# qgallouedec/deep_rl

Hardware: NVIDIA B200
Metric: PPO env-steps/sec (rollout+update) CartPole-v1 (higher is better)
Workload: dtype bf16

## Files before the change

deep_rl_b200/csrc/drl_env.cuh:

```cuda
#pragma once
#include "drl_common.cuh"

namespace drl {

template <int KIND> struct EnvSpec;
template <> struct EnvSpec<DRL_ENV_CARTPOLE> { static constexpr int O = 4, A = 2, OP = 4; };
template <> struct EnvSpec<DRL_ENV_ACROBOT>  { static constexpr int O = 6, A = 3, OP = 8; };
template <> struct EnvSpec<DRL_ENV_MOUNTAINCAR> { static constexpr int O = 2, A = 3, OP = 4; };

struct EnvLane {
    double s[4];
    int elapsed;
    float ep_ret;
    int ep_len;
};

__device__ __forceinline__ bool cartpole_physics(double (&s)[4], int action) {
    const double gravity = 9.8, masspole = 0.1, total_mass = 0.1 + 1.0, length = 0.5;
    const double polemass_length = 0.1 * 0.5, force_mag = 10.0, tau = 0.02;
    const double theta_thr = 12.0 * 2.0 * 3.14159265358979323846 / 360.0, x_thr = 2.4;
    double x = s[0], x_dot = s[1], th = s[2], th_dot = s[3];
    double force = action == 1 ? force_mag : -force_mag;
    double sinth, costh;
    sincos(th, &sinth, &costh);
    double temp = (force + polemass_length * (th_dot * th_dot) * sinth) / total_mass;
    double thacc = (gravity * sinth - costh * temp) / (length * (4.0 / 3.0 - masspole * (costh * costh) / total_mass));
    double xacc = temp - polemass_length * thacc * costh / total_mass;
    x = x + tau * x_dot;
    x_dot = x_dot + tau * xacc;
    th = th + tau * th_dot;
    th_dot = th_dot + tau * thacc;
    s[0] = x; s[1] = x_dot; s[2] = th; s[3] = th_dot;
    return (x < -x_thr) || (x > x_thr) || (th < -theta_thr) || (th > theta_thr);
}

__device__ __forceinline__ bool mountaincar_physics(double (&s)[4], int action) {
    double position = s[0], velocity = s[1];
    velocity = velocity + ((double)(action - 1) * 0.001 + cos(3.0 * position) * (-0.0025));
    velocity = fmin(fmax(velocity, -0.07), 0.07);
    position = position + velocity;
    position = fmin(fmax(position, -1.2), 0.6);
    if (position == -1.2 && velocity < 0.0) velocity = 0.0;
    s[0] = position; s[1] = velocity;
    return position >= 0.5 && velocity >= 0.0;
}

__device__ __forceinline__ void acrobot_dsdt(const double (&y)[4], double torque, double (&d)[4]) {
    const double m1 = 1.0, m2 = 1.0, l1 = 1.0, lc1 = 0.5, lc2 = 0.5, I1 = 1.0, I2 = 1.0, g = 9.8;
    const double PI = 3.14159265358979323846;
    double th1 = y[0], th2 = y[1], dth1 = y[2], dth2 = y[3];
    double s2, c2;
    sincos(th2, &s2, &c2);
    double d1 = m1 * (lc1 * lc1) + m2 * (l1 * l1 + lc2 * lc2 + 2.0 * l1 * lc2 * c2) + I1 + I2;
    double d2 = m2 * (lc2 * lc2 + l1 * lc2 * c2) + I2;
    double phi2 = m2 * lc2 * g * cos(th1 + th2 - PI / 2.0);
    double phi1 = -m2 * l1 * lc2 * (dth2 * dth2) * s2 - 2.0 * m2 * l1 * lc2 * dth2 * dth1 * s2 +
                  (m1 * lc1 + m2 * l1) * g * cos(th1 - PI / 2.0) + phi2;
    double ddth2 = (torque + d2 / d1 * phi1 - m2 * l1 * lc2 * (dth1 * dth1) * s2 - phi2) /
                   (m2 * (lc2 * lc2) + I2 - (d2 * d2) / d1);
    double ddth1 = -(d2 * ddth2 + phi1) / d1;
    d[0] = dth1; d[1] = dth2; d[2] = ddth1; d[3] = ddth2;
}

__device__ __forceinline__ double wrap_pi(double x) {
    const double PI = 3.14159265358979323846;
    const double diff = PI - (-PI);
    while (x > PI) x = x - diff;
    while (x < -PI) x = x + diff;
    return x;
}

__device__ __forceinline__ bool acrobot_physics(double (&s)[4], int action, float& reward) {
    const double PI = 3.14159265358979323846;
    const double dt = 0.2, dt2 = dt / 2.0;
    double torque = (double)action - 1.0;
    double k1[4], k2[4], k3[4], k4[4], yt[4];
    acrobot_dsdt(s, torque, k1);
#pragma unroll
    for (int i = 0; i < 4; ++i) yt[i] = s[i] + dt2 * k1[i];
    acrobot_dsdt(yt, torque, k2);
#pragma unroll
    for (int i = 0; i < 4; ++i) yt[i] = s[i] + dt2 * k2[i];
    acrobot_dsdt(yt, torque, k3);
#pragma unroll
    for (int i = 0; i < 4; ++i) yt[i] = s[i] + dt * k3[i];
    acrobot_dsdt(yt, torque, k4);
    double ns[4];
#pragma unroll
    for (int i = 0; i < 4; ++i) ns[i] = s[i] + dt / 6.0 * (k1[i] + 2.0 * k2[i] + 2.0 * k3[i] + k4[i]);
    ns[0] = wrap_pi(ns[0]);
    ns[1] = wrap_pi(ns[1]);
    ns[2] = fmin(fmax(ns[2], -4.0 * PI), 4.0 * PI);
    ns[3] = fmin(fmax(ns[3], -9.0 * PI), 9.0 * PI);
#pragma unroll
    for (int i = 0; i < 4; ++i) s[i] = ns[i];
    bool terminal = (-cos(ns[0]) - cos(ns[1] + ns[0])) > 1.0;
    reward = terminal ? 0.0f : -1.0f;
    return terminal;
}

template <int KIND>
__device__ __forceinline__ void env_observation(const double (&s)[4], float (&obs)[EnvSpec<KIND>::OP]) {
    if constexpr (KIND == DRL_ENV_CARTPOLE) {
#pragma unroll
        for (int i = 0; i < 4; ++i) obs[i] = (float)s[i];
    } else if constexpr (KIND == DRL_ENV_MOUNTAINCAR) {
        obs[0] = (float)s[0]; obs[1] = (float)s[1]; obs[2] = 0.0f; obs[3] = 0.0f;
    } else {
        double s1, c1, s2, c2;
        sincos(s[0], &s1, &c1);
        sincos(s[1], &s2, &c2);
        obs[0] = (float)c1; obs[1] = (float)s1; obs[2] = (float)c2; obs[3] = (float)s2;
        obs[4] = (float)s[2]; obs[5] = (float)s[3]; obs[6] = 0.0f; obs[7] = 0.0f;
    }
}

template <int KIND>
__device__ __forceinline__ void env_reset_state(double (&s)[4], uint64_t seed, uint32_t gid, uint64_t step) {
    uint4 o = philox_seeded(seed, gid, (uint32_t)step, (uint32_t)(step >> 32), TAG_RESET);
    if constexpr (KIND == DRL_ENV_MOUNTAINCAR) {
        s[0] = -0.6 + 0.2 * u01_f64(o.x);
        s[1] = 0.0; s[2] = 0.0; s[3] = 0.0;
        return;
    }
    const double half = KIND == DRL_ENV_CARTPOLE ? 0.05 : 0.1;
    s[0] = -half + (2.0 * half) * u01_f64(o.x);
    s[1] = -half + (2.0 * half) * u01_f64(o.y);
    s[2] = -half + (2.0 * half) * u01_f64(o.z);
    s[3] = -half + (2.0 * half) * u01_f64(o.w);
}

template <int KIND>
__device__ __forceinline__ bool env_physics(double (&s)[4], int action, float& reward) {
    if constexpr (KIND == DRL_ENV_CARTPOLE) { reward = 1.0f; return cartpole_physics(s, action); }
    else if constexpr (KIND == DRL_ENV_MOUNTAINCAR) { reward = -1.0f; return mountaincar_physics(s, action); }
    else { return acrobot_physics(s, action, reward); }
}

template <int KIND>
__device__ __forceinline__ bool env_after_physics(EnvLane& e, bool term, float reward, uint64_t seed, uint32_t gid, uint64_t step,
                                                  int max_episode_steps, const drl_ep_log_t& log);

template <int KIND>
__device__ __forceinline__ bool env_step(EnvLane& e, int action, float& reward, uint64_t seed, uint32_t gid,
                                         uint64_t step, int max_episode_steps, const drl_ep_log_t& log) {
    const bool term = env_physics<KIND>(e.s, action, reward);
    return env_after_physics<KIND>(e, term, reward, seed, gid, step, max_episode_steps, log);
}

template <int KIND>
__device__ __forceinline__ bool env_after_physics(EnvLane& e, bool term, float reward, uint64_t seed, uint32_t gid, uint64_t step,
                                                  int max_episode_steps, const drl_ep_log_t& log) {
    e.elapsed += 1;
    bool done = term || (e.elapsed >= max_episode_steps);
    e.ep_ret = e.ep_ret + reward;
    e.ep_len += 1;
    if (log.count != nullptr) {
        const unsigned active = __activemask();
        const unsigned dmask = __ballot_sync(active, done);
        if (dmask != 0u) {
            const int lane = (int)(threadIdx.x & 31u);
            const int leader = __ffs(dmask) - 1;
            double sr = 0.0, sl = 0.0;
            for (unsigned bits = dmask; bits != 0u; bits &= bits - 1u) {
                const int b = __ffs(bits) - 1;
                sr += (double)__shfl_sync(active, e.ep_ret, b);
                sl += (double)__shfl_sync(active, e.ep_len, b);
            }
            uint32_t base = 0;
            if (lane == leader) {
                base = atomicAdd(log.count, (uint32_t)__popc(dmask));
                if (log.sum_ret) atomicAdd(log.sum_ret, sr);
                if (log.sum_len) atomicAdd(log.sum_len, sl);
            }
            base = __shfl_sync(active, base, leader);
            if (done) {
                const uint32_t slot = base + (uint32_t)__popc(dmask & ((1u << lane) - 1u));
                if (slot < log.cap && log.entries) {
                    drl_ep_entry_t en;
                    en.step = step; en.env = gid; en.ret = e.ep_ret; en.len = e.ep_len; en.pad = 0u;
                    log.entries[slot] = en;
                }
            }
        }
    }
    if (done) {
        env_reset_state<KIND>(e.s, seed, gid, step);
        e.elapsed = 0; e.ep_ret = 0.0f; e.ep_len = 0;
    }
    return done;
}

__device__ __forceinline__ void env_load(EnvLane& e, const drl_env_t& env, int n) {
    const int N = env.num_envs;
#pragma unroll
    for (int i = 0; i < 4; ++i) e.s[i] = env.state[(size_t)i * N + n];
    e.elapsed = env.elapsed[n]; e.ep_ret = env.ep_ret[n]; e.ep_len = env.ep_len[n];
}
__device__ __forceinline__ void env_store(const EnvLane& e, const drl_env_t& env, int n) {
    const int N = env.num_envs;
#pragma unroll
    for (int i = 0; i < 4; ++i) env.state[(size_t)i * N + n] = e.s[i];
    env.elapsed[n] = e.elapsed; env.ep_ret[n] = e.ep_ret; env.ep_len[n] = e.ep_len;
}

}
```

deep_rl_b200/csrc/rollout_tc.cu:

```cuda
#include "drl_env.cuh"
#include "drl_pack.cuh"
#include "drl_tc_common.cuh"

namespace drl {

int check_env(const drl_env_t* env);
drl_ep_log_t log_or_empty(const drl_ep_log_t* log);

#ifdef DRL_ROLLOUT_STAMPS
__device__ long long g_ro_dbg[1024];
#define RO_STAMP(ev) do { if (blockIdx.x == 0 && lane == 0 && t >= 8 && t < 12 && (warp == 0 || warp == 5)) g_ro_dbg[(warp == 0 ? 0 : 512) + (t - 8) * 16 + (ev)] = clock64(); } while (0)
#else
#define RO_STAMP(ev) do { } while (0)
#endif
enum : uint32_t { RB_FWD = 1, RB_ROW0 = 2, RB_ROW1 = 6, RB_L1 = 10 };

template <int O, int A>
struct RoTcSmem {
    using P = Packed<O, A>;
    static constexpr int W_BYTES = (P::TC_END - P::TC_W2) * 4;
    static constexpr int OFF_W = 0;
    static constexpr int OFF_H1 = (OFF_W + W_BYTES + 1023) / 1024 * 1024;
    static constexpr int OFF_OBS = OFF_H1 + 32768;
    static constexpr int OBS_BYTES = TC_TILE * P::OW * 4 > 4096 ? TC_TILE * P::OW * 4 : 4096;
    static constexpr int OFF_XCH = OFF_OBS + OBS_BYTES;
    static constexpr int OFF_ST = OFF_XCH + 32 * TC_TILE * 4;
    static constexpr int OFF_CAND = OFF_ST + TC_TILE * 32;
    static constexpr int OFF_BAR = OFF_CAND + 3 * TC_TILE * 32 + 3 * TC_TILE * 8;
    static constexpr int TOTAL = OFF_BAR + 64 + 1024;
};

constexpr int RO_ENV_WARPS = 4;
constexpr int RO_THREADS = TC_THREADS + 32 * RO_ENV_WARPS;

template <int KIND, int REP>
__global__ void __launch_bounds__(RO_THREADS, 1) rollout_tc_kernel(drl_env_t env, const float* __restrict__ packed, int T,
                                                                   uint64_t step0, drl_rollout_buf_t buf, drl_ep_log_t log, const drl_ctrl_t* __restrict__ ctrl) {
    if (ctrl != nullptr) step0 = ctrl->env_step;
    using SP = EnvSpec<KIND>;
    constexpr int O = SP::O, A = SP::A, OP = SP::OP;
    using P = Packed<O, A>;
    using S = RoTcSmem<O, A>;
    constexpr int OW = P::OW;
    constexpr int ROWS = TC_TILE / REP;
    constexpr int QG = 4 / REP;
    constexpr int UPT = HU / REP;
    constexpr bool SPECULATE = KIND != DRL_ENV_ACROBOT;
    static_assert(OW == OP, "obs stride");
    static_assert(REP == 1 || REP == 2 || REP == 4, "replication factor");
    extern __shared__ unsigned char smem_raw[];
    unsigned char* sm = smem_raw + ((1024u - (smem_u32(smem_raw) & 1023u)) & 1023u);
    unsigned char* tW2 = sm + S::OFF_W;
    const float* sW1 = reinterpret_cast<const float*>(sm + S::OFF_W + 2 * H * H * 2);
    const float* sB1 = sW1 + 2 * H * OW;
    const float* sB2 = sB1 + 2 * H;
    const float* sW4 = sB2 + 2 * H;
    const float* sB4 = sW4 + (A + 1) * H;
    unsigned char* tH1 = sm + S::OFF_H1;
    float* obs_s = reinterpret_cast<float*>(sm + S::OFF_OBS);
    float* xch = reinterpret_cast<float*>(sm + S::OFF_XCH);
    double* st_s = reinterpret_cast<double*>(sm + S::OFF_ST);
    double* cand_s = reinterpret_cast<double*>(sm + S::OFF_CAND);
    float2* cand_rt = reinterpret_cast<float2*>(sm + S::OFF_CAND + 3 * TC_TILE * 32);
    uint64_t* bars = reinterpret_cast<uint64_t*>(sm + S::OFF_BAR);
    uint32_t* slot = reinterpret_cast<uint32_t*>(bars + 3);
    unsigned char* tW1B = reinterpret_cast<unsigned char*>(const_cast<float*>(sB4 + 4));
    unsigned char* tOBS = sm + S::OFF_OBS;

    const int tid = threadIdx.x, warp = tid >> 5, lane = tid & 31;
    const bool is_mma_warp = warp == TC_COMPUTE / 32;

    if (tid == 0) {
        mbar_init(bars, 1);
        mbar_init(bars + 1, 1);
        mbar_init(bars + 2, 1);
        mbar_fence_init();
    }
    if (is_mma_warp) umma::tmem_alloc(slot, 128);
    umma::fence_before_sync();
    __syncthreads();
    umma::fence_after_sync();
    if (tid == 0) {
        mbar_expect_tx(bars, (uint32_t)S::W_BYTES);
        const char* src = reinterpret_cast<const char*>(packed + P::TC_W2);
        for (uint32_t off = 0; off < (uint32_t)S::W_BYTES; off += 16384u) {
            const uint32_t n = (uint32_t)S::W_BYTES - off < 16384u ? (uint32_t)S::W_BYTES - off : 16384u;
            bulk_g2s(sm + S::OFF_W + off, src + off, n, bars);
        }
    }
    const uint32_t tmem = *slot;
    mbar_wait(bars, 0);

    if (is_mma_warp) {
        const uint32_t aW2 = smem_u32(tW2), aH1 = smem_u32(tH1);
        constexpr uint32_t ID_FWD = umma::make_idesc(128, 64, false, false);
        const uint32_t aW1B = smem_u32(tW1B), aOBS = smem_u32(tOBS);
        constexpr uint32_t ID_L1 = umma::make_idesc(128, 64, false, false);
        for (int t = 0; t <= T; ++t) {
            if (REP == 1) {
                named_bar_sync(RB_L1, 128 + 32);
                umma::fence_after_sync();
                if (umma::elect_one()) {
#pragma unroll
                    for (int n2 = 0; n2 < 2; ++n2)
                        umma::mma(tmem + n2 * 64, umma::make_desc(aOBS, 2048, 128, umma::LAYOUT_NONE),
                                  umma::make_desc(aW1B + n2 * 2048, 1024, 128, umma::LAYOUT_NONE), ID_L1, 0u);
                    umma::commit(bars + 2);
                }
                __syncwarp();
            }
            named_bar_sync(RB_FWD, TC_THREADS);
            umma::fence_after_sync();
            if (umma::elect_one()) {
#pragma unroll
                for (int n2 = 0; n2 < 2; ++n2)
#pragma unroll
                    for (int kb = 0; kb < 4; ++kb)
                        umma::mma(tmem + n2 * 64, umma::make_desc(aH1 + n2 * 16384 + kb * 32, 16, 1024, umma::LAYOUT_SW128),
                                  umma::make_desc(aW2 + n2 * 8192 + kb * 32, 16, 1024, umma::LAYOUT_SW128), ID_FWD, kb > 0);
                umma::commit(bars + 1);
            }
            __syncwarp();
        }
        umma::fence_before_sync();
        __syncthreads();
        umma::tmem_dealloc(tmem, 128);
        return;
    }

    if (warp > TC_COMPUTE / 32) {
        const int eg = warp - TC_COMPUTE / 32 - 1;
        if (eg < ROWS / 32) {
            const int er_e = eg * 32 + lane;
            const bool live = blockIdx.x * ROWS + er_e < env.num_envs;
            for (int t = 0; t <= T; ++t) {
                named_bar_sync(RB_ROW0 + eg, 128 * REP + 32);
                if (SPECULATE && t < T && live) {
                    const double2* sp = reinterpret_cast<const double2*>(st_s + er_e * 4);
                    const double2 s01 = sp[0], s23 = sp[1];
#pragma unroll
                    for (int a = 0; a < A; ++a) {
                        double cs[4] = {s01.x, s01.y, s23.x, s23.y};
                        float creward;
                        const bool cterm = env_physics<KIND>(cs, a, creward);
                        double2* cp = reinterpret_cast<double2*>(cand_s + ((size_t)a * TC_TILE + er_e) * 4);
                        cp[0] = make_double2(cs[0], cs[1]);
                        cp[1] = make_double2(cs[2], cs[3]);
                        cand_rt[a * TC_TILE + er_e] = make_float2(creward, cterm ? 1.0f : 0.0f);
                    }
                }
                named_bar_arrive(RB_ROW1 + eg, 128 * REP + 32);
            }
        }
        umma::fence_before_sync();
        __syncthreads();
        return;
    }

    const int q = warp & 3, half = (warp >> 2) & 1, net = (warp >> 3) & 1;
    const int grp = q % QG, replica = q / QG;
    const int er = grp * 32 + lane;
    const int u0 = half * HU + replica * UPT;
    const uint32_t trow = tmem + ((uint32_t)(q * 32) << 16);
    const int wrow0 = net == 0 ? 0 : A;
    const int nheads = net == 0 ? A : 1;
    const bool owner_warp = net == 0 && half == 0 && replica == 0;
    const int N = env.num_envs;
    const int n = blockIdx.x * ROWS + er;
    const bool own = owner_warp && n < N;
    const uint32_t gid = env.env_gid0 + (uint32_t)n;
    constexpr int NSLOT = 2 * REP;

    EnvLane e;
    e.s[0] = e.s[1] = e.s[2] = e.s[3] = 0.0; e.elapsed = 0; e.ep_ret = 0.0f; e.ep_len = 0;
    if (own) env_load(e, env, n);
    float lp_diff = 0.0f, lp_sum = 1.0f;

    for (int t = 0; t <= T; ++t) {
        RO_STAMP(0);

        if (owner_warp) {
            float obs[OP];
#pragma unroll
            for (int i = 0; i < OP; ++i) obs[i] = 0.0f;
            if (own) {
                env_observation<KIND>(e.s, obs);
                float4* o4 = reinterpret_cast<float4*>(buf.obs + ((size_t)t * N + n) * OP);
#pragma unroll
                for (int qq = 0; qq < OP / 4; ++qq) o4[qq] = make_float4(obs[4 * qq], obs[4 * qq + 1], obs[4 * qq + 2], obs[4 * qq + 3]);
                double2* sp = reinterpret_cast<double2*>(st_s + er * 4);
                sp[0] = make_double2(e.s[0], e.s[1]);
                sp[1] = make_double2(e.s[2], e.s[3]);
            }
            if (REP == 1) {
                float o16[16];
#pragma unroll
                for (int i = 0; i < 16; ++i) o16[i] = 0.0f;
#pragma unroll
                for (int i = 0; i < O; ++i) {
                    const float hi = __bfloat162float(__float2bfloat16_rn(obs[i]));
                    o16[i] = hi;
                    o16[8 + i] = obs[i] - hi;
                }
                o16[O] = 1.0f;
                umma::store_row_ns16(tOBS, TC_TILE, er, o16);
                umma::fence_proxy_async();
                umma::fence_before_sync();
                named_bar_arrive(RB_L1, 128 + 32);
            } else {
#pragma unroll
                for (int i = 0; i < OP; ++i) {
                    const float hi = __bfloat162float(__float2bfloat16_rn(obs[i]));
                    obs[i] = hi + __bfloat162float(__float2bfloat16_rn(obs[i] - hi));
                }
#pragma unroll
                for (int qq = 0; qq < OP / 4; ++qq)
                    *reinterpret_cast<float4*>(obs_s + er * OW + 4 * qq) = make_float4(obs[4 * qq], obs[4 * qq + 1], obs[4 * qq + 2], obs[4 * qq + 3]);
            }
        }
        RO_STAMP(1);
        named_bar_sync(RB_ROW0 + grp, 128 * REP + 32);
        RO_STAMP(2);

        if (REP == 1) {
            mbar_wait(bars + 2, (uint32_t)t & 1u);
            umma::fence_after_sync();
            float h[UPT];
            umma::ldn<UPT>(trow + net * 64 + u0, h);
#pragma unroll
            for (int j = 0; j < UPT; ++j) h[j] = tanh_mufu(h[j]);
#pragma unroll
            for (int c = 0; c < UPT / 8; ++c) {
                uint4 ch;
                ch.x = umma::pack_bf16(h[8 * c + 0], h[8 * c + 1]);
                ch.y = umma::pack_bf16(h[8 * c + 2], h[8 * c + 3]);
                ch.z = umma::pack_bf16(h[8 * c + 4], h[8 * c + 5]);
                ch.w = umma::pack_bf16(h[8 * c + 6], h[8 * c + 7]);
                *reinterpret_cast<uint4*>(tH1 + net * 16384 + umma::sw128_off(q * 32 + lane, u0 / 8 + c)) = ch;
            }
        } else {
            float x[OW];
#pragma unroll
            for (int qq = 0; qq < OW / 4; ++qq) {
                const float4 v4 = *reinterpret_cast<const float4*>(obs_s + er * OW + 4 * qq);
                x[4 * qq] = v4.x; x[4 * qq + 1] = v4.y; x[4 * qq + 2] = v4.z; x[4 * qq + 3] = v4.w;
            }
            float h[UPT];
            const float* w1 = sW1 + (net * H + u0) * OW;
            const float* b1 = sB1 + net * H + u0;
#pragma unroll
            for (int k4 = 0; k4 < UPT / 4; ++k4) {
                const float4 bb = *reinterpret_cast<const float4*>(b1 + 4 * k4);
                const float bv[4] = {bb.x, bb.y, bb.z, bb.w};
#pragma unroll
                for (int j = 0; j < 4; ++j) {
                    const int kk = 4 * k4 + j;
                    float z = bv[j];
#pragma unroll
                    for (int qq = 0; qq < OW / 4; ++qq) {
                        const float4 w = *reinterpret_cast<const float4*>(w1 + kk * OW + 4 * qq);
                        z = fmaf(x[4 * qq + 3], w.w, fmaf(x[4 * qq + 2], w.z, fmaf(x[4 * qq + 1], w.y, fmaf(x[4 * qq], w.x, z))));
                    }
                    h[kk] = tanh_mufu(z);
                }
            }
            uint4 ch[UPT / 8];
#pragma unroll
            for (int c = 0; c < UPT / 8; ++c) {
                ch[c].x = umma::pack_bf16(h[8 * c + 0], h[8 * c + 1]);
                ch[c].y = umma::pack_bf16(h[8 * c + 2], h[8 * c + 3]);
                ch[c].z = umma::pack_bf16(h[8 * c + 4], h[8 * c + 5]);
                ch[c].w = umma::pack_bf16(h[8 * c + 6], h[8 * c + 7]);
            }
#pragma unroll
            for (int rp = 0; rp < REP; ++rp) {
                const int row = (rp * QG + grp) * 32 + lane;
#pragma unroll
                for (int c = 0; c < UPT / 8; ++c)
                    *reinterpret_cast<uint4*>(tH1 + net * 16384 + umma::sw128_off(row, u0 / 8 + c)) = ch[c];
            }
        }
        RO_STAMP(3);
        umma::fence_proxy_async();
        umma::fence_before_sync();
        named_bar_arrive(RB_FWD, TC_THREADS);
        RO_STAMP(4);

        uint4 rr = make_uint4(0u, 0u, 0u, 0u);
        if (own) {
            if (t > 0) buf.logp[(size_t)(t - 1) * N + n] = __fsub_rn(lp_diff, logf(lp_sum));
            if (t < T) {
                const uint64_t step = step0 + (uint64_t)t;
                rr = philox_seeded(env.seed, gid, (uint32_t)step, (uint32_t)(step >> 32), TAG_ACTION);
            }
        }

        mbar_wait(bars + 1, (uint32_t)t & 1u);
        umma::fence_after_sync();
        RO_STAMP(5);
        {
            float h[UPT];
            umma::ldn<UPT>(trow + net * 64 + u0, h);
            const float* b2 = sB2 + net * H + u0;
#pragma unroll
            for (int k4 = 0; k4 < UPT / 4; ++k4) {
                const float4 bb = *reinterpret_cast<const float4*>(b2 + 4 * k4);
                h[4 * k4 + 0] = tanh_mufu(h[4 * k4 + 0] + bb.x);
                h[4 * k4 + 1] = tanh_mufu(h[4 * k4 + 1] + bb.y);
                h[4 * k4 + 2] = tanh_mufu(h[4 * k4 + 2] + bb.z);
                h[4 * k4 + 3] = tanh_mufu(h[4 * k4 + 3] + bb.w);
            }
#pragma unroll
            for (int a = 0; a < A; ++a) {
                if (a < nheads) {
                    const float* w = sW4 + (wrow0 + a) * H + u0;
                    float s0 = 0.f, s1 = 0.f, s2 = 0.f, s3 = 0.f;
#pragma unroll
                    for (int k4 = 0; k4 < UPT / 4; ++k4) {
                        const float4 ww = *reinterpret_cast<const float4*>(w + 4 * k4);
                        s0 = fmaf(h[4 * k4 + 0], ww.x, s0);
                        s1 = fmaf(h[4 * k4 + 1], ww.y, s1);
                        s2 = fmaf(h[4 * k4 + 2], ww.z, s2);
                        s3 = fmaf(h[4 * k4 + 3], ww.w, s3);
                    }
                    const int j = half * REP + replica;
                    const int sl = net == 0 ? j * A + a : NSLOT * A + j;
                    xch[sl * TC_TILE + er] = (s0 + s1) + (s2 + s3);
                }
            }
        }
        RO_STAMP(6);
        umma::fence_before_sync();
        named_bar_sync(RB_ROW1 + grp, 128 * REP + 32);
        RO_STAMP(7);

        if (own) {
            const size_t i0 = (size_t)t * N + n;
            float v = xch[(NSLOT * A) * TC_TILE + er];
#pragma unroll
            for (int j = 1; j < NSLOT; ++j) v += xch[(NSLOT * A + j) * TC_TILE + er];
            buf.val[i0] = v + sB4[A];
            if (t < T) {
                float l[A];
#pragma unroll
                for (int a = 0; a < A; ++a) {
                    float sacc = xch[a * TC_TILE + er];
#pragma unroll
                    for (int j = 1; j < NSLOT; ++j) sacc += xch[(j * A + a) * TC_TILE + er];
                    l[a] = sacc + sB4[a];
                }
                if (buf.logits != nullptr) {
#pragma unroll
                    for (int a = 0; a < A; ++a) buf.logits[i0 * A + a] = l[a];
                }
                RO_STAMP(8);
                const uint64_t step = step0 + (uint64_t)t;
                RO_STAMP(9);
                const int act = sample_categorical_split<A>(l, u01_f32(rr.x), lp_diff, lp_sum);
                RO_STAMP(10);
                buf.act[i0] = (uint8_t)act;
                float reward;
                bool term;
                if (SPECULATE) {
                    const double2* cp = reinterpret_cast<const double2*>(cand_s + ((size_t)act * TC_TILE + er) * 4);
                    const double2 c01 = cp[0], c23 = cp[1];
                    e.s[0] = c01.x; e.s[1] = c01.y; e.s[2] = c23.x; e.s[3] = c23.y;
                    const float2 rt = cand_rt[act * TC_TILE + er];
                    reward = rt.x; term = rt.y != 0.0f;
                } else {
                    term = env_physics<KIND>(e.s, act, reward);
                }
                const bool done = env_after_physics<KIND>(e, term, reward, env.seed, gid, step, env.max_episode_steps, log);
                buf.rew[i0 + N] = reward;
                buf.done[i0 + N] = done ? 1 : 0;
                RO_STAMP(11);
            }
        }
    }
    if (own) env_store(e, env, n);
    umma::fence_before_sync();
    __syncthreads();
}

template <int KIND, int REP>
static int launch_rollout_tc_rep(const drl_env_t& env, const float* packed, int T, uint64_t step0, const drl_rollout_buf_t& buf,
                                 const drl_ep_log_t& log, cudaStream_t st, const drl_ctrl_t* ctrl) {
    using SP = EnvSpec<KIND>;
    const int smem = RoTcSmem<SP::O, SP::A>::TOTAL;
    DRL_CUDA(cudaFuncSetAttribute(rollout_tc_kernel<KIND, REP>, cudaFuncAttributeMaxDynamicSharedMemorySize, smem));
    constexpr int ROWS = TC_TILE / REP;
    const int blocks = (env.num_envs + ROWS - 1) / ROWS;
    rollout_tc_kernel<KIND, REP><<<blocks, RO_THREADS, smem, st>>>(env, packed, T, step0, buf, log, ctrl);
    DRL_LAUNCH_CHECK("rollout_tc_kernel");
    return DRL_OK;
}

template <int KIND>
static int launch_rollout_tc_kind(const drl_env_t& env, const float* packed, int T, uint64_t step0, const drl_rollout_buf_t& buf,
                                  const drl_ep_log_t& log, cudaStream_t st, const drl_ctrl_t* ctrl) {
    const int sms = sm_count();
    int rows = 128;
    if ((env.num_envs + 127) / 128 < sms) rows = (env.num_envs + 63) / 64 <= sms ? 64 : 128;
    if ((env.num_envs + 63) / 64 < sms && (env.num_envs + 31) / 32 <= sms) rows = 32;
    const char* ov = getenv("DRL_ROLLOUT_ROWS");
    if (ov) { const int v = atoi(ov); if (v == 32 || v == 64 || v == 128) rows = v; }
    if (rows == 32) return launch_rollout_tc_rep<KIND, 4>(env, packed, T, step0, buf, log, st, ctrl);
    if (rows == 64) return launch_rollout_tc_rep<KIND, 2>(env, packed, T, step0, buf, log, st, ctrl);
    return launch_rollout_tc_rep<KIND, 1>(env, packed, T, step0, buf, log, st, ctrl);
}

int launch_rollout_tc(const drl_env_t& env, const float* packed, int T, uint64_t step0, const drl_rollout_buf_t& buf,
                      const drl_ep_log_t& log, cudaStream_t st, const drl_ctrl_t* ctrl) {
    if (env.kind == DRL_ENV_CARTPOLE) return launch_rollout_tc_kind<DRL_ENV_CARTPOLE>(env, packed, T, step0, buf, log, st, ctrl);
    if (env.kind == DRL_ENV_MOUNTAINCAR) return launch_rollout_tc_kind<DRL_ENV_MOUNTAINCAR>(env, packed, T, step0, buf, log, st, ctrl);
    return launch_rollout_tc_kind<DRL_ENV_ACROBOT>(env, packed, T, step0, buf, log, st, ctrl);
}

}

#ifdef DRL_ROLLOUT_STAMPS
extern "C" int drl_debug_rollout_stamps(long long* host_out) {
    return cudaMemcpyFromSymbol(host_out, drl::g_ro_dbg, sizeof(long long) * 1024) == cudaSuccess ? 0 : 1;
}
#endif
```

Before: 545.1 million.

## Speculatively run forward pass on all candidate next states in REP=4 rollout

For CartPole and MountainCar with 32-row tiles, the env warps now precompute the next state for every possible action. They write each candidate observation to shared memory, and the MMA warp then runs layer 2 for all candidates at once into a larger TMEM allocation. Once the action is sampled, compute warps just select the matching hidden row, which takes env physics and layer 1 off the serial per-step critical path. Env warps are split into three roles: sampling, candidate stepping, and bookkeeping/log writes. The cost is NC times more layer-1/MMA work, more shared memory and TMEM, and extra barriers.

```diff
diff --git a/deep_rl_b200/csrc/drl_env.cuh b/deep_rl_b200/csrc/drl_env.cuh
--- a/deep_rl_b200/csrc/drl_env.cuh
+++ b/deep_rl_b200/csrc/drl_env.cuh
@@ -148,11 +148,7 @@
     return env_after_physics<KIND>(e, term, reward, seed, gid, step, max_episode_steps, log);
 }
 
-template <int KIND>
-__device__ __forceinline__ bool env_after_physics(EnvLane& e, bool term, float reward, uint64_t seed, uint32_t gid, uint64_t step,
-                                                  int max_episode_steps, const drl_ep_log_t& log) {
-    e.elapsed += 1;
-    bool done = term || (e.elapsed >= max_episode_steps);
+__device__ __forceinline__ void env_record_step(EnvLane& e, bool done, float reward, uint32_t gid, uint64_t step, const drl_ep_log_t& log) {
     e.ep_ret = e.ep_ret + reward;
     e.ep_len += 1;
     if (log.count != nullptr) {
@@ -184,10 +180,28 @@
             }
         }
     }
+    if (done) { e.ep_ret = 0.0f; e.ep_len = 0; }
+}
+
+template <int KIND>
+__device__ __forceinline__ bool env_after_physics(EnvLane& e, bool term, float reward, uint64_t seed, uint32_t gid, uint64_t step,
+                                                  int max_episode_steps, const drl_ep_log_t& log) {
+    e.elapsed += 1;
+    const bool done = term || (e.elapsed >= max_episode_steps);
+    env_record_step(e, done, reward, gid, step, log);
     if (done) {
         env_reset_state<KIND>(e.s, seed, gid, step);
-        e.elapsed = 0; e.ep_ret = 0.0f; e.ep_len = 0;
-    }
+        e.elapsed = 0;
+    }
+    return done;
+}
+
+template <int KIND>
+__device__ __forceinline__ bool env_next_state(double (&s)[4], int action, int elapsed, int max_episode_steps, uint64_t seed,
+                                               uint32_t gid, uint64_t step, float& reward) {
+    const bool term = env_physics<KIND>(s, action, reward);
+    const bool done = term || (elapsed + 1 >= max_episode_steps);
+    if (done) env_reset_state<KIND>(s, seed, gid, step);
     return done;
 }
 
diff --git a/deep_rl_b200/csrc/rollout_tc.cu b/deep_rl_b200/csrc/rollout_tc.cu
--- a/deep_rl_b200/csrc/rollout_tc.cu
+++ b/deep_rl_b200/csrc/rollout_tc.cu
@@ -9,25 +9,30 @@
 
 #ifdef DRL_ROLLOUT_STAMPS
 __device__ long long g_ro_dbg[1024];
-#define RO_STAMP(ev) do { if (blockIdx.x == 0 && lane == 0 && t >= 8 && t < 12 && (warp == 0 || warp == 5)) g_ro_dbg[(warp == 0 ? 0 : 512) + (t - 8) * 16 + (ev)] = clock64(); } while (0)
+#define RO_STAMP(ev) do { if (blockIdx.x == 0 && lane == 0 && t >= 8 && t < 12 && (warp == 0 || warp == RO_STAMP_W2 || (SPEC && warp == RO_STAMP_W2 + 1))) g_ro_dbg[(warp == 0 ? 0 : 512) + (t - 8) * 16 + (ev)] = clock64(); } while (0)
 #else
 #define RO_STAMP(ev) do { } while (0)
 #endif
-enum : uint32_t { RB_FWD = 1, RB_ROW0 = 2, RB_ROW1 = 6, RB_L1 = 10 };
-
-template <int O, int A>
+enum : uint32_t { RB_FWD = 1, RB_ROW0 = 2, RB_ROW1 = 6, RB_L1 = 10, RB_ACT = 11 };
+
+template <int KIND, int REP>
+constexpr int ro_cands() { return KIND != DRL_ENV_ACROBOT && REP == 4 ? EnvSpec<KIND>::A : 1; }
+
+template <int O, int A, int NC>
 struct RoTcSmem {
     using P = Packed<O, A>;
     static constexpr int W_BYTES = (P::TC_END - P::TC_W2) * 4;
     static constexpr int OFF_W = 0;
     static constexpr int OFF_H1 = (OFF_W + W_BYTES + 1023) / 1024 * 1024;
-    static constexpr int OFF_OBS = OFF_H1 + 32768;
-    static constexpr int OBS_BYTES = TC_TILE * P::OW * 4 > 4096 ? TC_TILE * P::OW * 4 : 4096;
+    static constexpr int OFF_OBS = OFF_H1 + NC * 32768;
+    static constexpr int OBS_BYTES = NC > 1 ? 2 * NC * TC_TILE * P::OW * 4
+                                   : TC_TILE * P::OW * 4 > 4096 ? TC_TILE * P::OW * 4 : 4096;
     static constexpr int OFF_XCH = OFF_OBS + OBS_BYTES;
     static constexpr int OFF_ST = OFF_XCH + 32 * TC_TILE * 4;
     static constexpr int OFF_CAND = OFF_ST + TC_TILE * 32;
-    static constexpr int OFF_BAR = OFF_CAND + 3 * TC_TILE * 32 + 3 * TC_TILE * 8;
+    static constexpr int OFF_BAR = OFF_CAND + (NC > 1 ? 2 : 1) * (3 * TC_TILE * 32 + 3 * TC_TILE * 8);
     static constexpr int TOTAL = OFF_BAR + 64 + 1024;
+    static_assert(TOTAL <= 227 * 1024, "shared memory of one CTA");
 };
 
 constexpr int RO_ENV_WARPS = 4;
@@ -40,13 +45,18 @@
     using SP = EnvSpec<KIND>;
     constexpr int O = SP::O, A = SP::A, OP = SP::OP;
     using P = Packed<O, A>;
-    using S = RoTcSmem<O, A>;
+    constexpr int NC = ro_cands<KIND, REP>();
+    constexpr bool SPEC = NC > 1;
+    using S = RoTcSmem<O, A, NC>;
     constexpr int OW = P::OW;
     constexpr int ROWS = TC_TILE / REP;
     constexpr int QG = 4 / REP;
     constexpr int UPT = HU / REP;
     constexpr bool SPECULATE = KIND != DRL_ENV_ACROBOT;
     static_assert(OW == OP, "obs stride");
+    constexpr uint32_t TMEM_COLS = NC == 1 ? 128u : NC == 2 ? 256u : 512u;
+    constexpr int RO_STAMP_W2 = SPEC ? TC_COMPUTE / 32 + 1 : 5;
+    (void)RO_STAMP_W2;
     static_assert(REP == 1 || REP == 2 || REP == 4, "replication factor");
     extern __shared__ unsigned char smem_raw[];
     unsigned char* sm = smem_raw + ((1024u - (smem_u32(smem_raw) & 1023u)) & 1023u);
@@ -76,7 +86,7 @@
         mbar_init(bars + 2, 1);
         mbar_fence_init();
     }
-    if (is_mma_warp) umma::tmem_alloc(slot, 128);
+    if (is_mma_warp) umma::tmem_alloc(slot, TMEM_COLS);
     umma::fence_before_sync();
     __syncthreads();
     umma::fence_after_sync();
@@ -113,43 +123,205 @@
             umma::fence_after_sync();
             if (umma::elect_one()) {
 #pragma unroll
-                for (int n2 = 0; n2 < 2; ++n2)
-#pragma unroll
-                    for (int kb = 0; kb < 4; ++kb)
-                        umma::mma(tmem + n2 * 64, umma::make_desc(aH1 + n2 * 16384 + kb * 32, 16, 1024, umma::LAYOUT_SW128),
-                                  umma::make_desc(aW2 + n2 * 8192 + kb * 32, 16, 1024, umma::LAYOUT_SW128), ID_FWD, kb > 0);
+                for (int c = 0; c < NC; ++c)
+#pragma unroll
+                    for (int n2 = 0; n2 < 2; ++n2)
+#pragma unroll
+                        for (int kb = 0; kb < 4; ++kb)
+                            umma::mma(tmem + c * 128 + n2 * 64, umma::make_desc(aH1 + c * 32768 + n2 * 16384 + kb * 32, 16, 1024, umma::LAYOUT_SW128),
+                                      umma::make_desc(aW2 + n2 * 8192 + kb * 32, 16, 1024, umma::LAYOUT_SW128), ID_FWD, kb > 0);
                 umma::commit(bars + 1);
             }
             __syncwarp();
         }
         umma::fence_before_sync();
         __syncthreads();
-        umma::tmem_dealloc(tmem, 128);
+        umma::tmem_dealloc(tmem, TMEM_COLS);
         return;
     }
 
+    constexpr int NSLOT = 2 * REP;
+    constexpr uint32_t N_ACT = 128 * REP + 3 * 32;
+    const int N = env.num_envs;
+
+    auto round_hi_lo = [](float (&obs)[OP]) {
+#pragma unroll
+        for (int i = 0; i < OP; ++i) {
+            const float hi = __bfloat162float(__float2bfloat16_rn(obs[i]));
+            obs[i] = hi + __bfloat162float(__float2bfloat16_rn(obs[i] - hi));
+        }
+    };
+    auto store_obs_row = [](float* dst, const float (&obs)[OP]) {
+#pragma unroll
+        for (int qq = 0; qq < OP / 4; ++qq)
+            reinterpret_cast<float4*>(dst)[qq] = make_float4(obs[4 * qq], obs[4 * qq + 1], obs[4 * qq + 2], obs[4 * qq + 3]);
+    };
+    auto head_value = [&](int r) {
+        float v = xch[(NSLOT * A) * TC_TILE + r];
+#pragma unroll
+        for (int j = 1; j < NSLOT; ++j) v += xch[(NSLOT * A + j) * TC_TILE + r];
+        return v + sB4[A];
+    };
+    auto head_logits = [&](int r, float (&l)[A]) {
+#pragma unroll
+        for (int a = 0; a < A; ++a) {
+            float sacc = xch[a * TC_TILE + r];
+#pragma unroll
+            for (int j = 1; j < NSLOT; ++j) sacc += xch[(j * A + a) * TC_TILE + r];
+            l[a] = sacc + sB4[a];
+        }
+    };
+
     if (warp > TC_COMPUTE / 32) {
         const int eg = warp - TC_COMPUTE / 32 - 1;
-        if (eg < ROWS / 32) {
+        if constexpr (SPEC) {
+            const int n = blockIdx.x * ROWS + lane;
+            const bool live = blockIdx.x * ROWS + lane < env.num_envs;
+            const uint32_t gid = env.env_gid0 + (uint32_t)n;
+            int* sel_s = reinterpret_cast<int*>(st_s);
+            double2* cst = reinterpret_cast<double2*>(cand_s);
+            float2* crt = reinterpret_cast<float2*>(cand_s + 2 * NC * TC_TILE * 4);
+            if (eg == 0) {
+                float lp_diff = 0.0f, lp_sum = 1.0f;
+                sel_s[lane] = 0;
+                named_bar_arrive(RB_ACT, N_ACT);
+                for (int t = 0; t <= T; ++t) {
+                    const uint64_t step = step0 + (uint64_t)t;
+                    uint4 rr = make_uint4(0u, 0u, 0u, 0u);
+                    if (live && t < T) rr = philox_seeded(env.seed, gid, (uint32_t)step, (uint32_t)(step >> 32), TAG_ACTION);
+                    RO_STAMP(2);
+                    named_bar_sync(RB_ROW1, 128 * REP + 32);
+                    RO_STAMP(3);
+                    const size_t i0 = (size_t)t * N + n;
+                    int act = 0;
+                    float l[A];
+                    if (live && t < T) {
+                        head_logits(lane, l);
+                        act = sample_categorical_split<A>(l, u01_f32(rr.x), lp_diff, lp_sum);
+                        sel_s[((t + 1) & 1) * TC_TILE + lane] = act;
+                    }
+                    if (t < T) named_bar_arrive(RB_ACT, N_ACT);
+                    RO_STAMP(4);
+                    if (live) {
+                        buf.val[i0] = head_value(lane);
+                        if (t < T) {
+                            if (buf.logits != nullptr) {
+#pragma unroll
+                                for (int a = 0; a < A; ++a) buf.logits[i0 * A + a] = l[a];
+                            }
+                            buf.act[i0] = (uint8_t)act;
+                            buf.logp[i0] = __fsub_rn(lp_diff, logf(lp_sum));
+                        }
+                    }
+                }
+            } else if (eg == 1) {
+                double s[4] = {0.0, 0.0, 0.0, 0.0};
+                int elapsed = 0;
+                if (live) {
+#pragma unroll
+                    for (int i = 0; i < 4; ++i) s[i] = env.state[(size_t)i * N + n];
+                    elapsed = env.elapsed[n];
+                }
+                {
+                    float obs[OP];
+#pragma unroll
+                    for (int i = 0; i < OP; ++i) obs[i] = 0.0f;
+                    if (live) env_observation<KIND>(s, obs);
+                    round_hi_lo(obs);
+#pragma unroll
+                    for (int c = 0; c < NC; ++c) store_obs_row(obs_s + ((size_t)c * TC_TILE + lane) * OW, obs);
+                }
+                named_bar_arrive(RB_ROW0, 128 * REP + 32);
+                for (int t = 0; t <= T; ++t) {
+                    RO_STAMP(0);
+                    named_bar_sync(RB_ACT, N_ACT);
+                    RO_STAMP(1);
+                    if (t == T) break;
+                    const int par = t & 1, npar = (t + 1) & 1;
+                    if (live && t > 0) {
+                        const int c = sel_s[par * TC_TILE + lane];
+                        const double2* cp = cst + ((size_t)(par * NC + c) * TC_TILE + lane) * 2;
+                        const double2 c01 = cp[0], c23 = cp[1];
+                        s[0] = c01.x; s[1] = c01.y; s[2] = c23.x; s[3] = c23.y;
+                        elapsed = crt[(par * NC + c) * TC_TILE + lane].y != 0.0f ? 0 : elapsed + 1;
+                    }
+                    const uint64_t step = step0 + (uint64_t)t;
+#pragma unroll
+                    for (int c = 0; c < NC; ++c) {
+                        float obs[OP];
+#pragma unroll
+                        for (int i = 0; i < OP; ++i) obs[i] = 0.0f;
+                        if (live) {
+                            double cs[4] = {s[0], s[1], s[2], s[3]};
+                            float crew;
+                            const bool cdone = env_next_state<KIND>(cs, c, elapsed, env.max_episode_steps, env.seed, gid, step, crew);
+                            env_observation<KIND>(cs, obs);
+                            double2* cp = cst + ((size_t)(npar * NC + c) * TC_TILE + lane) * 2;
+                            cp[0] = make_double2(cs[0], cs[1]);
+                            cp[1] = make_double2(cs[2], cs[3]);
+                            crt[(npar * NC + c) * TC_TILE + lane] = make_float2(crew, cdone ? 1.0f : 0.0f);
+                        }
+                        round_hi_lo(obs);
+                        store_obs_row(obs_s + ((size_t)(npar * NC + c) * TC_TILE + lane) * OW, obs);
+                    }
+                    RO_STAMP(5);
+                    named_bar_arrive(RB_ROW0, 128 * REP + 32);
+                }
+            } else if (eg == 2) {
+                EnvLane e;
+                e.s[0] = e.s[1] = e.s[2] = e.s[3] = 0.0; e.elapsed = 0; e.ep_ret = 0.0f; e.ep_len = 0;
+                if (live) {
+                    env_load(e, env, n);
+                    float obs[OP];
+                    env_observation<KIND>(e.s, obs);
+                    store_obs_row(buf.obs + (size_t)n * OP, obs);
+                }
+                named_bar_sync(RB_ACT, N_ACT);
+                for (int t = 0; t < T; ++t) {
+                    named_bar_sync(RB_ACT, N_ACT);
+                    if (live) {
+                        const int par = (t + 1) & 1;
+                        const int c = sel_s[par * TC_TILE + lane];
+                        const double2* cp = cst + ((size_t)(par * NC + c) * TC_TILE + lane) * 2;
+                        const double2 c01 = cp[0], c23 = cp[1];
+                        const float2 rt = crt[(par * NC + c) * TC_TILE + lane];
+                        e.s[0] = c01.x; e.s[1] = c01.y; e.s[2] = c23.x; e.s[3] = c23.y;
+                        const float reward = rt.x;
+                        const bool done = rt.y != 0.0f;
+                        e.elapsed = done ? 0 : e.elapsed + 1;
+                        const size_t i1 = (size_t)(t + 1) * N + n;
+                        buf.rew[i1] = reward;
+                        buf.done[i1] = done ? 1 : 0;
+                        float obs[OP];
+                        env_observation<KIND>(e.s, obs);
+                        store_obs_row(buf.obs + i1 * OP, obs);
+                        env_record_step(e, done, reward, gid, step0 + (uint64_t)t, log);
+                    }
+                }
+                if (live) env_store(e, env, n);
+            }
+        } else if (eg < ROWS / 32) {
             const int er_e = eg * 32 + lane;
             const bool live = blockIdx.x * ROWS + er_e < env.num_envs;
-            for (int t = 0; t <= T; ++t) {
-                named_bar_sync(RB_ROW0 + eg, 128 * REP + 32);
-                if (SPECULATE && t < T && live) {
-                    const double2* sp = reinterpret_cast<const double2*>(st_s + er_e * 4);
-                    const double2 s01 = sp[0], s23 = sp[1];
-#pragma unroll
-                    for (int a = 0; a < A; ++a) {
-                        double cs[4] = {s01.x, s01.y, s23.x, s23.y};
-                        float creward;
-                        const bool cterm = env_physics<KIND>(cs, a, creward);
-                        double2* cp = reinterpret_cast<double2*>(cand_s + ((size_t)a * TC_TILE + er_e) * 4);
-                        cp[0] = make_double2(cs[0], cs[1]);
-                        cp[1] = make_double2(cs[2], cs[3]);
-                        cand_rt[a * TC_TILE + er_e] = make_float2(creward, cterm ? 1.0f : 0.0f);
+            {
+                for (int t = 0; t <= T; ++t) {
+                    named_bar_sync(RB_ROW0 + eg, 128 * REP + 32);
+                    if (SPECULATE && t < T && live) {
+                        const double2* sp = reinterpret_cast<const double2*>(st_s + er_e * 4);
+                        const double2 s01 = sp[0], s23 = sp[1];
+#pragma unroll
+                        for (int a = 0; a < A; ++a) {
+                            double cs[4] = {s01.x, s01.y, s23.x, s23.y};
+                            float creward;
+                            const bool cterm = env_physics<KIND>(cs, a, creward);
+                            double2* cp = reinterpret_cast<double2*>(cand_s + ((size_t)a * TC_TILE + er_e) * 4);
+                            cp[0] = make_double2(cs[0], cs[1]);
+                            cp[1] = make_double2(cs[2], cs[3]);
+                            cand_rt[a * TC_TILE + er_e] = make_float2(creward, cterm ? 1.0f : 0.0f);
+                        }
                     }
-                }
-                named_bar_arrive(RB_ROW1 + eg, 128 * REP + 32);
+                    named_bar_arrive(RB_ROW1 + eg, 128 * REP + 32);
+                }
             }
         }
         umma::fence_before_sync();
@@ -164,12 +336,119 @@
     const uint32_t trow = tmem + ((uint32_t)(q * 32) << 16);
     const int wrow0 = net == 0 ? 0 : A;
     const int nheads = net == 0 ? A : 1;
+
+    auto layer1_rows = [&](const float* x_row, unsigned char* h1) {
+        float x[OW];
+#pragma unroll
+        for (int qq = 0; qq < OW / 4; ++qq) {
+            const float4 v4 = *reinterpret_cast<const float4*>(x_row + 4 * qq);
+            x[4 * qq] = v4.x; x[4 * qq + 1] = v4.y; x[4 * qq + 2] = v4.z; x[4 * qq + 3] = v4.w;
+        }
+        float h[UPT];
+        const float* w1 = sW1 + (net * H + u0) * OW;
+        const float* b1 = sB1 + net * H + u0;
+#pragma unroll
+        for (int k4 = 0; k4 < UPT / 4; ++k4) {
+            const float4 bb = *reinterpret_cast<const float4*>(b1 + 4 * k4);
+            const float bv[4] = {bb.x, bb.y, bb.z, bb.w};
+#pragma unroll
+            for (int j = 0; j < 4; ++j) {
+                const int kk = 4 * k4 + j;
+                float z = bv[j];
+#pragma unroll
+                for (int qq = 0; qq < OW / 4; ++qq) {
+                    const float4 w = *reinterpret_cast<const float4*>(w1 + kk * OW + 4 * qq);
+                    z = fmaf(x[4 * qq + 3], w.w, fmaf(x[4 * qq + 2], w.z, fmaf(x[4 * qq + 1], w.y, fmaf(x[4 * qq], w.x, z))));
+                }
+                h[kk] = tanh_mufu(z);
+            }
+        }
+        uint4 ch[UPT / 8];
+#pragma unroll
+        for (int c = 0; c < UPT / 8; ++c) {
+            ch[c].x = umma::pack_bf16(h[8 * c + 0], h[8 * c + 1]);
+            ch[c].y = umma::pack_bf16(h[8 * c + 2], h[8 * c + 3]);
+            ch[c].z = umma::pack_bf16(h[8 * c + 4], h[8 * c + 5]);
+            ch[c].w = umma::pack_bf16(h[8 * c + 6], h[8 * c + 7]);
+        }
+#pragma unroll
+        for (int rp = 0; rp < REP; ++rp) {
+            const int row = (rp * QG + grp) * 32 + lane;
+#pragma unroll
+            for (int c = 0; c < UPT / 8; ++c)
+                *reinterpret_cast<uint4*>(h1 + net * 16384 + umma::sw128_off(row, u0 / 8 + c)) = ch[c];
+        }
+    };
+    auto head_partials = [&](float (&h)[UPT]) {
+        const float* b2 = sB2 + net * H + u0;
+#pragma unroll
+        for (int k4 = 0; k4 < UPT / 4; ++k4) {
+            const float4 bb = *reinterpret_cast<const float4*>(b2 + 4 * k4);
+            h[4 * k4 + 0] = tanh_mufu(h[4 * k4 + 0] + bb.x);
+            h[4 * k4 + 1] = tanh_mufu(h[4 * k4 + 1] + bb.y);
+            h[4 * k4 + 2] = tanh_mufu(h[4 * k4 + 2] + bb.z);
+            h[4 * k4 + 3] = tanh_mufu(h[4 * k4 + 3] + bb.w);
+        }
+#pragma unroll
+        for (int a = 0; a < A; ++a) {
+            if (a < nheads) {
+                const float* w = sW4 + (wrow0 + a) * H + u0;
+                float s0 = 0.f, s1 = 0.f, s2 = 0.f, s3 = 0.f;
+#pragma unroll
+                for (int k4 = 0; k4 < UPT / 4; ++k4) {
+                    const float4 ww = *reinterpret_cast<const float4*>(w + 4 * k4);
+                    s0 = fmaf(h[4 * k4 + 0], ww.x, s0);
+                    s1 = fmaf(h[4 * k4 + 1], ww.y, s1);
+                    s2 = fmaf(h[4 * k4 + 2], ww.z, s2);
+                    s3 = fmaf(h[4 * k4 + 3], ww.w, s3);
+                }
+                const int j = half * REP + replica;
+                const int sl = net == 0 ? j * A + a : NSLOT * A + j;
+                xch[sl * TC_TILE + er] = (s0 + s1) + (s2 + s3);
+            }
+        }
+    };
+
+    if constexpr (SPEC) {
+        const int* sel_s = reinterpret_cast<const int*>(st_s);
+        for (int t = 0; t <= T; ++t) {
+            RO_STAMP(6);
+            named_bar_sync(RB_ROW0 + grp, 128 * REP + 32);
+            RO_STAMP(7);
+#pragma unroll
+            for (int c = 0; c < NC; ++c) layer1_rows(obs_s + ((size_t)((t & 1) * NC + c) * TC_TILE + er) * OW, tH1 + c * 32768);
+            umma::fence_proxy_async();
+            umma::fence_before_sync();
+            named_bar_arrive(RB_FWD, TC_THREADS);
+            RO_STAMP(8);
+            named_bar_sync(RB_ACT, N_ACT);
+            const int sel = sel_s[(t & 1) * TC_TILE + er];
+            RO_STAMP(9);
+            mbar_wait(bars + 1, (uint32_t)t & 1u);
+            umma::fence_after_sync();
+            RO_STAMP(10);
+            float h[UPT];
+#pragma unroll
+            for (int c = 0; c < NC; ++c) {
+                float hc[UPT];
+                umma::ldn<UPT>(trow + c * 128 + net * 64 + u0, hc);
+#pragma unroll
+                for (int j = 0; j < UPT; ++j) h[j] = (c == 0 || c == sel) ? hc[j] : h[j];
+            }
+            head_partials(h);
+            umma::fence_before_sync();
+            named_bar_arrive(RB_ROW1 + grp, 128 * REP + 32);
+            RO_STAMP(11);
+        }
+        umma::fence_before_sync();
+        __syncthreads();
+        return;
+    }
+
     const bool owner_warp = net == 0 && half == 0 && replica == 0;
-    const int N = env.num_envs;
     const int n = blockIdx.x * ROWS + er;
     const bool own = owner_warp && n < N;
     const uint32_t gid = env.env_gid0 + (uint32_t)n;
-    constexpr int NSLOT = 2 * REP;
 
     EnvLane e;
     e.s[0] = e.s[1] = e.s[2] = e.s[3] = 0.0; e.elapsed = 0; e.ep_ret = 0.0f; e.ep_len = 0;
@@ -185,9 +464,7 @@
             for (int i = 0; i < OP; ++i) obs[i] = 0.0f;
             if (own) {
                 env_observation<KIND>(e.s, obs);
-                float4* o4 = reinterpret_cast<float4*>(buf.obs + ((size_t)t * N + n) * OP);
-#pragma unroll
-                for (int qq = 0; qq < OP / 4; ++qq) o4[qq] = make_float4(obs[4 * qq], obs[4 * qq + 1], obs[4 * qq + 2], obs[4 * qq + 3]);
+                store_obs_row(buf.obs + ((size_t)t * N + n) * OP, obs);
                 double2* sp = reinterpret_cast<double2*>(st_s + er * 4);
                 sp[0] = make_double2(e.s[0], e.s[1]);
                 sp[1] = make_double2(e.s[2], e.s[3]);
@@ -208,14 +485,8 @@
                 umma::fence_before_sync();
                 named_bar_arrive(RB_L1, 128 + 32);
             } else {
-#pragma unroll
-                for (int i = 0; i < OP; ++i) {
-                    const float hi = __bfloat162float(__float2bfloat16_rn(obs[i]));
-                    obs[i] = hi + __bfloat162float(__float2bfloat16_rn(obs[i] - hi));
-                }
-#pragma unroll
-                for (int qq = 0; qq < OP / 4; ++qq)
-                    *reinterpret_cast<float4*>(obs_s + er * OW + 4 * qq) = make_float4(obs[4 * qq], obs[4 * qq + 1], obs[4 * qq + 2], obs[4 * qq + 3]);
+                round_hi_lo(obs);
+                store_obs_row(obs_s + er * OW, obs);
             }
         }
         RO_STAMP(1);
@@ -239,46 +510,7 @@
                 *reinterpret_cast<uint4*>(tH1 + net * 16384 + umma::sw128_off(q * 32 + lane, u0 / 8 + c)) = ch;
             }
         } else {
-            float x[OW];
-#pragma unroll
-            for (int qq = 0; qq < OW / 4; ++qq) {
-                const float4 v4 = *reinterpret_cast<const float4*>(obs_s + er * OW + 4 * qq);
-                x[4 * qq] = v4.x; x[4 * qq + 1] = v4.y; x[4 * qq + 2] = v4.z; x[4 * qq + 3] = v4.w;
-            }
-            float h[UPT];
-            const float* w1 = sW1 + (net * H + u0) * OW;
-            const float* b1 = sB1 + net * H + u0;
-#pragma unroll
-            for (int k4 = 0; k4 < UPT / 4; ++k4) {
-                const float4 bb = *reinterpret_cast<const float4*>(b1 + 4 * k4);
-                const float bv[4] = {bb.x, bb.y, bb.z, bb.w};
-#pragma unroll
-                for (int j = 0; j < 4; ++j) {
-                    const int kk = 4 * k4 + j;
-                    float z = bv[j];
-#pragma unroll
-                    for (int qq = 0; qq < OW / 4; ++qq) {
-                        const float4 w = *reinterpret_cast<const float4*>(w1 + kk * OW + 4 * qq);
-                        z = fmaf(x[4 * qq + 3], w.w, fmaf(x[4 * qq + 2], w.z, fmaf(x[4 * qq + 1], w.y, fmaf(x[4 * qq], w.x, z))));
-                    }
-                    h[kk] = tanh_mufu(z);
-                }
-            }
-            uint4 ch[UPT / 8];
-#pragma unroll
-            for (int c = 0; c < UPT / 8; ++c) {
-                ch[c].x = umma::pack_bf16(h[8 * c + 0], h[8 * c + 1]);
-                ch[c].y = umma::pack_bf16(h[8 * c + 2], h[8 * c + 3]);
-                ch[c].z = umma::pack_bf16(h[8 * c + 4], h[8 * c + 5]);
-                ch[c].w = umma::pack_bf16(h[8 * c + 6], h[8 * c + 7]);
-            }
-#pragma unroll
-            for (int rp = 0; rp < REP; ++rp) {
-                const int row = (rp * QG + grp) * 32 + lane;
-#pragma unroll
-                for (int c = 0; c < UPT / 8; ++c)
-                    *reinterpret_cast<uint4*>(tH1 + net * 16384 + umma::sw128_off(row, u0 / 8 + c)) = ch[c];
-            }
+            layer1_rows(obs_s + er * OW, tH1);
         }
         RO_STAMP(3);
         umma::fence_proxy_async();
@@ -301,33 +533,7 @@
         {
             float h[UPT];
             umma::ldn<UPT>(trow + net * 64 + u0, h);
-            const float* b2 = sB2 + net * H + u0;
-#pragma unroll
-            for (int k4 = 0; k4 < UPT / 4; ++k4) {
-                const float4 bb = *reinterpret_cast<const float4*>(b2 + 4 * k4);
-                h[4 * k4 + 0] = tanh_mufu(h[4 * k4 + 0] + bb.x);
-                h[4 * k4 + 1] = tanh_mufu(h[4 * k4 + 1] + bb.y);
-                h[4 * k4 + 2] = tanh_mufu(h[4 * k4 + 2] + bb.z);
-                h[4 * k4 + 3] = tanh_mufu(h[4 * k4 + 3] + bb.w);
-            }
-#pragma unroll
-            for (int a = 0; a < A; ++a) {
-                if (a < nheads) {
-                    const float* w = sW4 + (wrow0 + a) * H + u0;
-                    float s0 = 0.f, s1 = 0.f, s2 = 0.f, s3 = 0.f;
-#pragma unroll
-                    for (int k4 = 0; k4 < UPT / 4; ++k4) {
-                        const float4 ww = *reinterpret_cast<const float4*>(w + 4 * k4);
-                        s0 = fmaf(h[4 * k4 + 0], ww.x, s0);
-                        s1 = fmaf(h[4 * k4 + 1], ww.y, s1);
-                        s2 = fmaf(h[4 * k4 + 2], ww.z, s2);
-                        s3 = fmaf(h[4 * k4 + 3], ww.w, s3);
-                    }
-                    const int j = half * REP + replica;
-                    const int sl = net == 0 ? j * A + a : NSLOT * A + j;
-                    xch[sl * TC_TILE + er] = (s0 + s1) + (s2 + s3);
-                }
-            }
+            head_partials(h);
         }
         RO_STAMP(6);
         umma::fence_before_sync();
@@ -336,19 +542,10 @@
 
         if (own) {
             const size_t i0 = (size_t)t * N + n;
-            float v = xch[(NSLOT * A) * TC_TILE + er];
-#pragma unroll
-            for (int j = 1; j < NSLOT; ++j) v += xch[(NSLOT * A + j) * TC_TILE + er];
-            buf.val[i0] = v + sB4[A];
+            buf.val[i0] = head_value(er);
             if (t < T) {
                 float l[A];
-#pragma unroll
-                for (int a = 0; a < A; ++a) {
-                    float sacc = xch[a * TC_TILE + er];
-#pragma unroll
-                    for (int j = 1; j < NSLOT; ++j) sacc += xch[(j * A + a) * TC_TILE + er];
-                    l[a] = sacc + sB4[a];
-                }
+                head_logits(er, l);
                 if (buf.logits != nullptr) {
 #pragma unroll
                     for (int a = 0; a < A; ++a) buf.logits[i0 * A + a] = l[a];
@@ -386,7 +583,7 @@
 static int launch_rollout_tc_rep(const drl_env_t& env, const float* packed, int T, uint64_t step0, const drl_rollout_buf_t& buf,
                                  const drl_ep_log_t& log, cudaStream_t st, const drl_ctrl_t* ctrl) {
     using SP = EnvSpec<KIND>;
-    const int smem = RoTcSmem<SP::O, SP::A>::TOTAL;
+    const int smem = RoTcSmem<SP::O, SP::A, ro_cands<KIND, REP>()>::TOTAL;
     DRL_CUDA(cudaFuncSetAttribute(rollout_tc_kernel<KIND, REP>, cudaFuncAttributeMaxDynamicSharedMemorySize, smem));
     constexpr int ROWS = TC_TILE / REP;
     const int blocks = (env.num_envs + ROWS - 1) / ROWS;
```

Measured after the change: 514.3 million (median of 6 runs). 0.944x the previous value.
